# wjwei-handsome/wgatools

Hardware: AMD Instinct MI355X
Metric: paf_cigar_ops_per_s (paf2maf+stat) (higher is better)
Workload: dtype u8

## Files before the change

wgatools_amd/csrc/capi_paf2maf.inc:

```
static inline u32 job_tiles_for(int param, u64 nt) {
  if (param >= 1) return param > (int)WGA_S_MAX_JOB_TILES ? WGA_S_MAX_JOB_TILES : (u32)param;
  return nt < 200000ull ? 4u : 8u;
}

extern "C" {

size_t wga_tile_ws_bytes(uint64_t n_ops) { return (size_t)(n_tiles(n_ops) * sizeof(wga_tile_sum)) + 16; }

int wga_cigar_stat(wga_ctx* c, const wga_cigar_batch* b, wga_cigar_counts* d_counts,
                   wga_rec_diag* d_diag, void* d_tile_ws) {
  int rc = ctx_bind(c);
  if (rc) return rc;
  if ((rc = check_batch(b))) return rc;
  if (b->n == 0) return WGA_OK;
  if (!d_counts || !d_diag) return fail(WGA_E_INVALID_ARG, "d_counts / d_diag null", nullptr);
  RT_CHECK(rt_memset(d_counts, 0, (size_t)b->n * sizeof(wga_cigar_counts), c->stream));
  RT_CHECK(rt_memset(d_diag, 0xFF, (size_t)b->n * sizeof(wga_rec_diag), c->stream));
  u64 nt = n_tiles(b->n_ops);
  if (nt == 0) return WGA_OK;
  void* ws;
  if ((rc = ctx_scratch(c, (size_t)nt * sizeof(wga_tile_rec), &ws))) return rc;
  wga_tile_rec* tile_rec = (wga_tile_rec*)ws;
  WGA_LAUNCH(k_tile_rec, (u32)((nt + 255) / 256), WGA_BLOCK, c->stream, (const u64*)b->d_op_off,
             b->d_strand_neg, b->n, (u64)b->n_ops, tile_rec);
  LAUNCH_CHECK();
  const u32 grid = (u32)((nt + 3) / 4);
  WGA_LAUNCH(k_cigar_stat, grid, WGA_BLOCK, c->stream, b->d_ops, (const u64*)b->d_op_off,
             b->d_strand_neg, b->n, (u64)b->n_ops, (const wga_tile_rec*)tile_rec, d_counts, d_diag,
             (wga_tile_sum*)d_tile_ws);
  LAUNCH_CHECK();
  return WGA_OK;
}

int wga_exclusive_scan_u64(wga_ctx* c, uint32_t n, const uint64_t* d_in, uint64_t* d_out) {
  int rc = ctx_bind(c);
  if (rc) return rc;
  if (!d_out || (n && !d_in)) return fail(WGA_E_INVALID_ARG, "null array", nullptr);
  ScanPlain f;
  f.in = (const u64*)d_in;
  return run_scan(c, f, n, (u64*)d_out);
}

int wga_paf2maf_layout(wga_ctx* c, uint32_t n, const wga_cigar_counts* d_counts,
                       const uint64_t* d_t_src_len, const uint64_t* d_q_src_len,
                       const uint32_t* d_pre_t, const uint32_t* d_pre_q, const uint32_t* d_post,
                       uint64_t* d_t_row_off, uint64_t* d_q_row_off, uint64_t* d_rec_off) {
  int rc = ctx_bind(c);
  if (rc) return rc;
  if (!d_rec_off) return fail(WGA_E_INVALID_ARG, "d_rec_off null", nullptr);
  if (n && (!d_counts || !d_t_src_len || !d_q_src_len || !d_t_row_off || !d_q_row_off))
    return fail(WGA_E_INVALID_ARG, "null array", nullptr);
  ScanLayout f;
  f.counts = d_counts;
  f.t_src_len = (const u64*)d_t_src_len;
  f.q_src_len = (const u64*)d_q_src_len;
  f.pre_t = d_pre_t;
  f.pre_q = d_pre_q;
  f.post = d_post;
  rc = run_scan(c, f, n, (u64*)d_rec_off);
  if (rc) return rc;
  if (n) {
    WGA_LAUNCH(k_layout_rows, (n + 255u) / 256u, WGA_BLOCK, c->stream, f, n, (const u64*)d_rec_off,
               (u64*)d_t_row_off, (u64*)d_q_row_off);
    LAUNCH_CHECK();
  }
  return WGA_OK;
}

int wga_paf2maf_expand(wga_ctx* c, const wga_cigar_batch* b, const wga_cigar_counts* d_counts,
                       const void* d_tile_ws, const uint8_t* d_t_fa, uint64_t t_fa_bytes,
                       const uint64_t* d_t_src_off, const uint64_t* d_t_src_len,
                       const uint8_t* d_q_fa, uint64_t q_fa_bytes, const uint64_t* d_q_src_off,
                       const uint64_t* d_q_src_len, uint8_t* d_out, const uint64_t* d_t_row_off,
                       const uint64_t* d_q_row_off, wga_rec_diag* d_diag) {
  int rc = ctx_bind(c);
  if (rc) return rc;
  if ((rc = check_batch(b))) return rc;
  if (b->n == 0 || b->n_ops == 0) return WGA_OK;
  if (!d_counts || !d_tile_ws || !d_t_src_off || !d_t_src_len || !d_q_src_off || !d_q_src_len ||
      !d_out || !d_t_row_off || !d_q_row_off || !d_diag)
    return fail(WGA_E_INVALID_ARG, "null array", nullptr);
  if ((t_fa_bytes && !d_t_fa) || (q_fa_bytes && !d_q_fa)) return fail(WGA_E_INVALID_ARG, "null sequence pool", nullptr);
  u64 nt = n_tiles(b->n_ops);
  if (nt > 0x7FFFFFFFull) return fail(WGA_E_INVALID_ARG, "batch too large for one launch", nullptr);
  void* ws;
  size_t rec_bytes = ((size_t)b->n * sizeof(wga_rec_desc) + 255) & ~(size_t)255;
  const size_t desc_bytes = (size_t)nt * sizeof(wga_tile_desc);
  const size_t list_bytes = 2 * (size_t)nt * sizeof(u32);
  const int variant = c->expand_variant >= 0 ? c->expand_variant : WGA_AUTO_LONG_VARIANT;
  c->expand_variant_used = variant;
  const bool stream = variant == 3;
  const u32 job_tiles = job_tiles_for(c->expand_job_tiles, nt);
  const u64 jobs = (nt + job_tiles - 1) / job_tiles;
  const size_t flag_bytes = stream ? (((size_t)nt + 255) & ~(size_t)255) : 0;
  const size_t skip_bytes = stream ? (((size_t)jobs * sizeof(u32) + 255) & ~(size_t)255) : 0;
  const size_t zero_bytes = 256 + flag_bytes + skip_bytes;
  if ((rc = ctx_scratch(c, rec_bytes + desc_bytes + list_bytes + zero_bytes, &ws))) return rc;
  wga_rec_desc* recs = (wga_rec_desc*)ws;
  wga_tile_desc* tdesc = (wga_tile_desc*)((char*)ws + rec_bytes);
  u32* const wide_list = (u32*)((char*)ws + rec_bytes + desc_bytes);
  u32* const fast_list = wide_list + nt;
  u32* const wide_counts = (u32*)((char*)ws + rec_bytes + desc_bytes + list_bytes);
  u8* const tile_flag = stream ? (u8*)wide_counts + 256 : nullptr;
  u32* const job_skip = stream ? (u32*)(tile_flag + flag_bytes) : nullptr;
  if (stream) RT_CHECK(rt_memset(wide_counts, 0, zero_bytes, c->stream));
  WGA_LAUNCH(k_rec_desc, (b->n + 255u) / 256u, WGA_BLOCK, c->stream, b->n, d_counts,
             b->d_strand_neg, (const u64*)d_t_src_off, (const u64*)d_t_src_len,
             (const u64*)d_q_src_off, (const u64*)d_q_src_len, (const u64*)d_t_row_off,
             (const u64*)d_q_row_off, recs, (const u64*)b->d_op_off, (u64)t_fa_bytes, (u64)q_fa_bytes, tile_flag);
  LAUNCH_CHECK();
  WGA_LAUNCH(k_tile_base, (u32)((nt + 255) / 256), WGA_BLOCK, c->stream, (const u64*)b->d_op_off,
             (u64)b->n_ops, (const wga_tile_sum*)d_tile_ws, (const wga_rec_desc*)recs, tdesc, 0, (const u8*)tile_flag,
             job_tiles, c->expand_force_slow, job_skip, wide_counts, fast_list, wide_list);
  LAUNCH_CHECK();
  if (stream) c->stream_counts = wide_counts;
  ExpandArgs a;
  a.ops = b->d_ops;
  a.op_off = (const u64*)b->d_op_off;
  a.n_ops = b->n_ops;
  a.tdesc = tdesc;
  a.recs = recs;
  a.t_fa = d_t_fa;
  a.t_fa_bytes = t_fa_bytes;
  a.q_fa = d_q_fa;
  a.q_fa_bytes = q_fa_bytes;
  a.out = d_out;
  a.diag = d_diag;
  a.force_slow = c->expand_force_slow;
  a.no_table = c->expand_no_table;
  a.drain_min = 0;
  a.tile_count = nullptr;
  a.tile_list = nullptr;
  a.n_rec = b->n;
  a.job_tiles = job_tiles;
  a.job_skip = job_skip;
  a.drain_min = c->expand_drain_min ? c->expand_drain_min : ((u64)t_fa_bytes + (u64)q_fa_bytes > WGA_DRAIN_POOL_BYTES ? 16u : 32u);
  c->expand_drain_min_used = a.drain_min;
  const uint32_t slot = c->ev_n % (uint32_t)wga_ctx::kTimingRing;
  if (c->timing) RT_CHECK(rt_event_record(c->ev[2 * slot], c->stream));
  if (stream) {
    WGA_LAUNCH(k_paf2maf_expand_s, (u32)jobs, 128u, c->stream, a);
    LAUNCH_CHECK();
    const u32 side_grid = nt < 256 ? (u32)nt : 256u;
    a.tile_count = wide_counts;
    a.tile_list = fast_list;
    WGA_LAUNCH(k_paf2maf_expand_list, side_grid, WGA_BLOCK, c->stream, a);
    LAUNCH_CHECK();
    a.force_slow = 1;
    a.tile_count = wide_counts + 1;
    a.tile_list = wide_list;
    WGA_LAUNCH(k_paf2maf_expand_list, side_grid, WGA_BLOCK, c->stream, a);
    LAUNCH_CHECK();
  } else {
    WGA_LAUNCH(k_paf2maf_expand, (u32)nt, WGA_BLOCK, c->stream, a);
    LAUNCH_CHECK();
  }
  if (c->timing) {
    RT_CHECK(rt_event_record(c->ev[2 * slot + 1], c->stream));
    c->ev_n++;
  }
  return WGA_OK;
}

int wga_ctx_expand_timing(wga_ctx* c, double* ms_sum, uint32_t* launches) {
  int rc = ctx_bind(c);
  if (rc) return rc;
  if (!ms_sum || !launches) return fail(WGA_E_INVALID_ARG, "null argument", nullptr);
  *ms_sum = 0.0;
  *launches = 0;
  if (!c->timing) return WGA_OK;
  const uint32_t n = c->ev_n < (uint32_t)wga_ctx::kTimingRing ? c->ev_n : (uint32_t)wga_ctx::kTimingRing;
  for (uint32_t k = 0; k < n; k++) {
    float ms = 0.0f;
    RT_CHECK(rt_event_elapsed_ms(c->ev[2 * k], c->ev[2 * k + 1], &ms));
    *ms_sum += (double)ms;
  }
  *launches = n;
  c->ev_n = 0;
  return WGA_OK;
}

int wga_scatter_bytes(wga_ctx* c, uint32_t n, const uint8_t* d_src, const uint64_t* d_src_off,
                      uint8_t* d_dst, const uint64_t* d_dst_off) {
  int rc = ctx_bind(c);
  if (rc) return rc;
  if (n == 0) return WGA_OK;
  if (!d_src || !d_src_off || !d_dst || !d_dst_off) return fail(WGA_E_INVALID_ARG, "null array", nullptr);
  WGA_LAUNCH(k_scatter_bytes, (n + 3u) / 4u, WGA_BLOCK, c->stream, n, d_src, (const u64*)d_src_off,
             d_dst, (const u64*)d_dst_off);
  LAUNCH_CHECK();
  return WGA_OK;
}

int wga_counts_total(wga_ctx* c, uint32_t n, const wga_cigar_counts* d_counts, uint64_t* d_totals) {
  int rc = ctx_bind(c);
  if (rc) return rc;
  if (!d_totals || (n && !d_counts)) return fail(WGA_E_INVALID_ARG, "null array", nullptr);
  static_assert(sizeof(wga_cigar_counts) == 88, "wga_cigar_counts is 11 u64");
  RT_CHECK(rt_memset(d_totals, 0, 88, c->stream));
  if (n == 0) return WGA_OK;
  u32 grid = (u32)(((u64)n * 11ull + 253ull * 8ull - 1ull) / (253ull * 8ull));
  if (grid > 2048u) grid = 2048u;
  WGA_LAUNCH(k_counts_total, grid, WGA_BLOCK, c->stream, n, (const u64*)d_counts, (u64*)d_totals);
// ... 6 lines not shown
```

wgatools_amd/csrc/capi_pafpseudo.inc:

```
static CallKey class_tab_key(const wga_cigar_batch* b) {
  return {6, {{b->d_ops, (size_t)b->n_ops * 4}, {b->d_op_off, ((size_t)b->n + 1) * 8}}, {b->n, b->n_ops}};
}

extern "C" {

int wga_cigar_class_sums(wga_ctx* c, const wga_cigar_batch* b, wga_class_sums* d_sums) {
  int rc = ctx_bind(c);
  if (rc) return rc;
  if ((rc = check_batch(b))) return rc;
  if (b->n == 0) return WGA_OK;
  if (!d_sums) return fail(WGA_E_INVALID_ARG, "d_sums null", nullptr);
  wga_ctx::ClassTab& t = c->class_tab;
  const CallKey key = class_tab_key(b);
  t.cache.take(key, false);
  u64 nt = n_tiles(b->n_ops);
  if (nt == 0) {
    RT_CHECK(rt_memset(d_sums, 0, (size_t)b->n * sizeof(wga_class_sums), c->stream));
    return WGA_OK;
  }
  const size_t tile_bytes = ((size_t)nt * sizeof(wga_tile_sum) + 63) & ~(size_t)63;
  const size_t need = tile_bytes + (size_t)b->n * sizeof(wga_class_sums);
  if ((rc = t.buf.reserve(c, need, need + need / 4))) return rc;
  t.tiles = (wga_tile_sum*)t.buf.mem;
  t.rec_sums = (wga_class_sums*)((char*)t.buf.mem + tile_bytes);
// ... 24 lines not shown
  RT_CHECK(rt_memset(d_diag, 0xFF, (size_t)b->n * sizeof(wga_rec_diag), c->stream));
  u64 nt = n_tiles(b->n_ops);
  if (nt == 0) return WGA_OK;
  wga_tile_sum* tiles;
  wga_class_sums* rec_sums;
  wga_ctx::ClassTab& t = c->class_tab;
  const bool kept = t.cache.take(class_tab_key(b), true);
  if (nt > 0x7FFFFFFFull) return fail(WGA_E_INVALID_ARG, "batch too large for one launch", nullptr);
  const bool stream = c->pseudo_variant == 3;
  const size_t tile_bytes = kept ? 0 : ((size_t)nt * sizeof(wga_tile_sum) + 255) & ~(size_t)255;
  const size_t sums_bytes = kept ? 0 : ((size_t)b->n * sizeof(wga_class_sums) + 255) & ~(size_t)255;
  const size_t rec_bytes = stream ? ((size_t)b->n * sizeof(wga_rec_desc) + 255) & ~(size_t)255 : 0;
  const size_t desc_bytes = stream ? (size_t)nt * sizeof(wga_tile_desc) : 0;
  const size_t list_bytes = stream ? 2 * (size_t)nt * sizeof(u32) : 0;
  const u32 job_tiles = job_tiles_for(c->expand_job_tiles, nt);
  const u64 jobs = (nt + job_tiles - 1) / job_tiles;
  const size_t flag_bytes = stream ? (((size_t)nt + 255) & ~(size_t)255) : 0;
  const size_t skip_bytes = stream ? (((size_t)jobs * sizeof(u32) + 255) & ~(size_t)255) : 0;
  const size_t zero_bytes = stream ? 256 + flag_bytes + skip_bytes : 0;
  void* ws = nullptr;
  if (tile_bytes + sums_bytes + rec_bytes + desc_bytes + list_bytes + zero_bytes)
    if ((rc = ctx_scratch(c, tile_bytes + sums_bytes + rec_bytes + desc_bytes + list_bytes + zero_bytes, &ws))) return rc;
  c->pseudo_counts = nullptr;
  if (kept) {
    tiles = t.tiles;
    rec_sums = t.rec_sums;
  } else {
    tiles = (wga_tile_sum*)ws;
    rec_sums = (wga_class_sums*)((char*)ws + tile_bytes);
    RT_CHECK(rt_memset(rec_sums, 0, (size_t)b->n * sizeof(wga_class_sums), c->stream));
    WGA_LAUNCH(k_class_tiles, (u32)((nt + 3) / 4), WGA_BLOCK, c->stream, b->d_ops,
               (const u64*)b->d_op_off, b->n, (u64)b->n_ops, tiles, rec_sums);
    LAUNCH_CHECK();
  }
  PseudoArgs a;
  a.ops = b->d_ops;
  a.op_off = (const u64*)b->d_op_off;
  a.strand_neg = b->d_strand_neg;
  a.n = b->n;
  a.n_ops = b->n_ops;
  a.tiles = tiles;
  a.rec_sums = rec_sums;
  a.base_mode = base_mode;
  a.q_fa = d_q_fa;
  a.q_fa_bytes = q_fa_bytes;
  a.q_src_off = (const u64*)d_q_src_off;
  a.q_src_len = (const u64*)d_q_src_len;
  a.skip = (const u64*)d_skip;
  a.out = d_out;
  a.dst_off = (const u64*)d_dst_off;
  a.diag = d_diag;
  a.tile_count = nullptr;
  a.tile_list = nullptr;
  if (stream) {
    char* const base = (char*)ws + tile_bytes + sums_bytes;
    wga_rec_desc* const recs = (wga_rec_desc*)base;
    wga_tile_desc* const tdesc = (wga_tile_desc*)(base + rec_bytes);
    u32* const list_wide = (u32*)(base + rec_bytes + desc_bytes);
    u32* const list_fast = list_wide + nt;
    u32* const counts = (u32*)(base + rec_bytes + desc_bytes + list_bytes);
    u8* const tile_flag = (u8*)counts + 256;
    u32* const job_skip = (u32*)(tile_flag + flag_bytes);
    RT_CHECK(rt_memset(counts, 0, zero_bytes, c->stream));
    WGA_LAUNCH(k_pseudo_rec_desc, (b->n + 255u) / 256u, WGA_BLOCK, c->stream, b->n, (const wga_class_sums*)rec_sums, b->d_strand_neg,
               base_mode ? (const u64*)d_q_src_off : nullptr, base_mode ? (const u64*)d_q_src_len : nullptr, (const u64*)d_skip,
               (const u64*)d_dst_off, (const u64*)b->d_op_off, (u64)q_fa_bytes, recs, tile_flag);
    LAUNCH_CHECK();
    WGA_LAUNCH(k_tile_base, (u32)((nt + 255) / 256), WGA_BLOCK, c->stream, (const u64*)b->d_op_off, (u64)b->n_ops,
               (const wga_tile_sum*)tiles, (const wga_rec_desc*)recs, tdesc, 1, (const u8*)tile_flag, job_tiles, 0, job_skip, counts,
               list_fast, list_wide);
    LAUNCH_CHECK();
    c->pseudo_counts = counts;
    ExpandArgs e;
    memset(&e, 0, sizeof(e));
    e.ops = b->d_ops;
    e.op_off = (const u64*)b->d_op_off;
    e.n_ops = b->n_ops;
    e.tdesc = tdesc;
    e.recs = recs;
    e.q_fa = base_mode ? d_q_fa : nullptr;
    e.q_fa_bytes = base_mode ? q_fa_bytes : 0;
    e.out = d_out;
    e.diag = d_diag;
    e.n_rec = b->n;
    e.job_tiles = job_tiles;
    e.job_skip = job_skip;
    if (base_mode)
      WGA_LAUNCH(k_pafpseudo_stream, (u32)((jobs + 1) / 2), 128u, c->stream, e);
    else
      WGA_LAUNCH(k_pafpseudo_stream_sym, (u32)((jobs + 1) / 2), 128u, c->stream, e);
    LAUNCH_CHECK();
    const u32 side_grid = nt < 256 ? (u32)nt : 256u;
    a.tile_count = counts;
    a.tile_list = list_fast;
    if (base_mode)
      WGA_LAUNCH(k_pafpseudo_fill_list<true>, side_grid, WGA_BLOCK, c->stream, a);
    else
      WGA_LAUNCH(k_pafpseudo_fill_list<false>, side_grid, WGA_BLOCK, c->stream, a);
    LAUNCH_CHECK();
    a.tile_count = counts + 1;
    a.tile_list = list_wide;
    if (base_mode)
      WGA_LAUNCH(k_pafpseudo_fill_list<true>, side_grid, WGA_BLOCK, c->stream, a);
    else
      WGA_LAUNCH(k_pafpseudo_fill_list<false>, side_grid, WGA_BLOCK, c->stream, a);
    LAUNCH_CHECK();
    return WGA_OK;
  }
  if (base_mode)
    WGA_LAUNCH(k_pafpseudo_fill<true>, (u32)nt, WGA_BLOCK, c->stream, a);
  else
    WGA_LAUNCH(k_pafpseudo_fill<false>, (u32)nt, WGA_BLOCK, c->stream, a);
  LAUNCH_CHECK();
  return WGA_OK;
}

}
```

wgatools_amd/csrc/wga_k6_pafpseudo.h:

```cpp
#ifndef WGA_K6_PAFPSEUDO_H
#define WGA_K6_PAFPSEUDO_H

#include "wga_kernels.h"

struct PseudoArgs {
  const u32* ops;
  const u64* op_off;
  const u8* strand_neg;
  u32 n;
  u64 n_ops;
  const wga_tile_sum* tiles;
  const wga_class_sums* rec_sums;
  int base_mode;
  const u8* q_fa;
  u64 q_fa_bytes;
  const u64* q_src_off;
  const u64* q_src_len;
  const u64* skip;
  u8* out;
  const u64* dst_off;
  wga_rec_diag* diag;
  const u32* tile_count;
  const u32* tile_list;
};

__device__ __forceinline__ u32 pseudo_symbol(u32 code) {
  return (code == WGA_OP_M || code == WGA_OP_EQ)
             ? 0x31313131u
             : code == WGA_OP_X ? 0x30303030u
                                : (code == WGA_OP_D || code == WGA_OP_D_CONT) ? 0x2D2D2D2Du : 0u;
}

__device__ __forceinline__ void emit_symbols(u8* dst, u32 N, u32 c0, const u32* s_col,
                                             const u32* s_sym, int ka, int kb, const u32* optbl, u32 gsh,
                                             const u32x4_a16* lowmask, u32 tid, u32 nthreads) {
  if (N == 0) return;
  const u64 A = (u64)dst, E = A + N;
  const u64 first = A >> 4, last = (E - 1) >> 4;
  for (u64 ch = first + tid; ch <= last; ch += nthreads) {
    const u64 base_addr = ch << 4;
    const u32 a0 = base_addr < A ? (u32)(A - base_addr) : 0u;
    const u32 b0 = base_addr + 16 > E ? (u32)(E - base_addr) : 16u;
    const u32 cz = c0 + (u32)(base_addr - A);
    u32 c = cz + a0;
    const u32 c_end = cz + b0;
    (void)kb;
    int k = (int)optbl[c >> gsh] - 1;
    k = k < ka ? ka : k;
    u32 o[4] = {0u, 0u, 0u, 0u};
    while (c < c_end) {
      u32 oe = s_col[k + 1];
      u32 pe = oe < c_end ? oe : c_end;
      if (pe > c) {
        const u32 sym = s_sym[k];
        const u32 W[4] = {sym, sym, sym, sym};
        merge16(o, W, (int)(c - cz), (int)(pe - cz), lowmask);
        c = pe;
      }
      k++;
    }
    if (a0 == 0u && b0 == 16u) {
      u32x4_a16 v = {o[0], o[1], o[2], o[3]};
      *(u32x4_a16*)base_addr = v;
    } else {
      u8* p = (u8*)base_addr;
      for (u32 j = a0; j < b0; j++) {
        u32 d = j >> 2;
        u32 word = d == 0 ? o[0] : d == 1 ? o[1] : d == 2 ? o[2] : o[3];
        p[j] = (u8)(word >> (8u * (j & 3u)));
      }
    }
  }
}

#ifndef WGA_K6_BLOCKS_BASE
#define WGA_K6_BLOCKS_BASE 4
// ... 200 lines not shown
          rd.tsh = 0u;
          rd.gsh = gsh;
          rd.queue = s_queue;
          rowsrc_prepare(qs, qb);
          emit_row(dst + (x0 - skip), (u32)(x1 - x0), c_first, rd, qs, tid, WGA_BLOCK, bad_base);
        } else
          emit_symbols(dst + (x0 - skip), (u32)(x1 - x0), c_first, s_col, s_sym, (int)ka, (int)kb, s_tbl, gsh,
                       s_lowmask, tid, WGA_BLOCK);
      }
    }
    if (!fast) {
      u64 x = cb, qp = qb;
      for (u64 k = cur; k < seg_end; k++) {
        const u32 op = a.ops[k];
        const u32 code = op & 15u;
        const u32 c = op_class(code);
        const u64 len = op >> 4;
        if (BASE && tid == 0) {
          if ((c == CLS_I || c == CLS_S) && qp + len > qs.src_len) atomicMin(panic_idx, k - rs);
          if (c == CLS_D && qp > qs.src_len) atomicMin(panic_idx, k - rs);
        }
        if (c == CLS_MX || c == CLS_D) {
          for (u64 j = tid; j < len; j += WGA_BLOCK) {
            u64 xx = x + j;
            if (xx >= skip && xx < row_len) {
              u8 v;
              if (BASE)
                v = (c == CLS_D) ? (u8)'-' : src_byte(qs, qp + j, bad_base);
              else
                v = (u8)(pseudo_symbol(code) & 0xFFu);
              dst[xx - skip] = v;
            }
          }
          x += len;
        }
        if (c == CLS_MX || c == CLS_I || c == CLS_S) qp += len;
      }
    }
    if (seg_end == re && BASE && row_len > T_total) {
      u64 x0 = T_total > skip ? T_total : skip;
      if (row_len > x0)
        emit_tail(dst + (x0 - skip), row_len - x0, Q_total + (x0 - T_total), qs, s_lowmask, s_queue, s_zero2, s_g_col, tid, WGA_BLOCK, bad_base);
    }
    cur = seg_end;
    r++;
  }
}
template <bool BASE>
__global__ __launch_bounds__(256, BASE ? WGA_K6_BLOCKS_BASE : WGA_K6_BLOCKS_SYM) void k_pafpseudo_fill(PseudoArgs a) {
  pseudo_tile<BASE>(a, xcd_tile_of_block());
}
template <bool BASE>
__global__ __launch_bounds__(256, BASE ? WGA_K6_BLOCKS_BASE : WGA_K6_BLOCKS_SYM) void k_pafpseudo_fill_list(PseudoArgs a) {
  const u32 n_list = *a.tile_count;
  for (u32 idx = blockIdx.x; idx < n_list; idx += gridDim.x) {
    pseudo_tile<BASE>(a, a.tile_list[idx]);
    __syncthreads();
  }
}

#endif
```

wgatools_amd/csrc/wga_kernels.h:

```cpp
#ifndef WGA_KERNELS_H
#define WGA_KERNELS_H

#include "../../include/wga_hip.h"
#include "wga_rt.h"

typedef unsigned int u32;
typedef unsigned long long u64;
typedef long long i64;
typedef unsigned char u8;

#define WGA_TILE 1024u
#define WGA_BLOCK 256u
#define WGA_FAST_COL_LIMIT 0x7FFFFFFFull

#define CLS_MX 0u
#define CLS_I 1u
#define CLS_D 2u
#define CLS_S 3u
#define CLS_O 4u

__device__ __forceinline__ u32 op_class(u32 code) {
  const u64 lut = (u64)CLS_MX | ((u64)CLS_I << 3) | ((u64)CLS_D << 6) | ((u64)CLS_O << 9) |
                  ((u64)CLS_S << 12) | ((u64)CLS_O << 15) | ((u64)CLS_O << 18) |
                  ((u64)CLS_MX << 21) | ((u64)CLS_MX << 24) | ((u64)CLS_I << 27) |
// ... 55 lines not shown
  }
  return v;
}

__device__ __forceinline__ void block_excl_scan4_u32(const u32 v[4], u32 ex[4], u32 tot[4],
                                                     u32* s_w4, bool s_w4_idle = false) {
  const u32 lane = threadIdx.x & 63u, wave = WGA_WAVE_ID(threadIdx.x);
  u32 inc[4];
#pragma unroll
  for (int k = 0; k < 4; k++) inc[k] = wave_incl_scan_u32(v[k]);
  if (!s_w4_idle) __syncthreads();
  if (lane == 63u) {
#pragma unroll
    for (int k = 0; k < 4; k++) s_w4[wave * 4 + k] = inc[k];
  }
  __syncthreads();
#pragma unroll
  for (int k = 0; k < 4; k++) {
    u32 pre = 0, t = 0;
#pragma unroll
    for (u32 w = 0; w < 4; w++) {
      const u32 x = s_w4[w * 4 + k];
      pre += w < wave ? x : 0u;
      t += x;
    }
    ex[k] = pre + inc[k] - v[k];
    tot[k] = t;
  }
}

__device__ __forceinline__ u32 wga_find_rec(const u64* off, u32 n, u64 x) {
  u32 lane = threadIdx.x & 63u;
  u64 lo = 0, hi = (u64)n + 1;
  while (hi - lo > 1) {
    u64 span = hi - lo;
    u64 step = (span + 63) >> 6;
    u64 p = lo + (u64)(lane + 1) * step;
    int pred = (p < hi) && (off[p] <= x);
    u64 m = __ballot(pred);
    u64 k = (u64)__popcll(m);
    u64 nhi = lo + (k + 1) * step;
    lo = lo + k * step;
    hi = nhi < hi ? nhi : hi;
  }
  return (u32)lo;
}

struct wga_tile_rec {
  u32 rec, neg;
  u64 rs, re;
};
__global__ __launch_bounds__(256) void k_tile_rec(const u64* __restrict__ op_off,
                                                  const u8* __restrict__ strand_neg, u32 n, u64 n_ops,
                                                  wga_tile_rec* __restrict__ tile_rec) {
  const u64 g = (u64)blockIdx.x * 256 + threadIdx.x;
  const u64 x = g * WGA_TILE;
  if (x >= n_ops) return;
  u32 lo = 0, hi = n;
  while (hi - lo > 1u) {
    const u32 mid = lo + ((hi - lo) >> 1);
    if (op_off[mid] <= x)
      lo = mid;
    else
      hi = mid;
  }
  wga_tile_rec t;
  t.rec = lo;
  t.neg = strand_neg[lo] != 0 ? 1u : 0u;
  t.rs = op_off[lo];
  t.re = op_off[lo + 1];
  tile_rec[g] = t;
}

__device__ __forceinline__ void cigar_stat_tile(const u64 g, const u32 (&w)[16], const u32 lane, const u64* __restrict__ op_off,
                                                const u8* __restrict__ strand_neg, u64 n_ops,
                                                const wga_tile_rec* __restrict__ tile_rec, wga_cigar_counts* counts,
                                                wga_rec_diag* diag, wga_tile_sum* tiles) {
  const u64 tile_start = g * WGA_TILE;
  const u64 tile_end = tile_start + WGA_TILE < n_ops ? tile_start + WGA_TILE : n_ops;

  const wga_tile_rec tr = tile_rec[g];
  u32 r = WGA_UNI32(tr.rec);
  const u32 r_first = r;
  u64 cur = tile_start;
  u64 tot[5] = {0, 0, 0, 0, 0}, tail[5] = {0, 0, 0, 0, 0};
  u64 re = WGA_UNI64(tr.re);
  constexpr u32 MX_BITS = 0x01810181u, I_BITS = 0x02020202u, X_BITS = 0x01000100u, RARE_BITS = 0xF878F878u;
  constexpr u32 IEV_BITS = 0x00020002u, DEV_BITS = 0x00040004u;
  const u32 lane4 = lane * 4u;
  auto wave_sums = [&](u32 s_mx, u32 s_i, u32 s_t, u32 s_x, u32 ev, u64& Smx, u64& Si, u64& St, u64& Sx, u32& EV) {
    if (__ballot(s_t >= (1u << 26)) == 0ull) {
      Smx = wave_sum_u32(s_mx), Si = wave_sum_u32(s_i), St = wave_sum_u32(s_t), Sx = wave_sum_u32(s_x);
    } else {
      Smx = wave_sum_u32_wide(s_mx), Si = wave_sum_u32_wide(s_i), St = wave_sum_u32_wide(s_t), Sx = wave_sum_u32_wide(s_x);
    }
    EV = wave_sum_u32(ev);
  };
  u64 Wmx, Wi, Wt, Wx;
  u32 Wev;
  bool rare_tile;
  {
    u32 s_mx = 0, s_i = 0, s_t = 0, s_x = 0, ev = 0, rare = 0;
#pragma unroll
    for (int k = 0; k < 16; k++) {
      const u32 op = w[k], len = op >> 4;
      s_mx += len & bit_mask(MX_BITS, op);
      s_i += len & bit_mask(I_BITS, op);
      s_t += len;
// ... 248 lines not shown

template <typename F>
__global__ __launch_bounds__(256) void k_scan_partials(F f, u32 n, u64* partial) {
  __shared__ u64 s_w[5];
  u32 base = blockIdx.x * 1024u + threadIdx.x * 4u;
  u64 v = 0;
  for (u32 e = 0; e < 4; e++)
    if (base + e < n) v += f(base + e);
  u64 tot;
  (void)block_excl_scan_u64(v, s_w, &tot);
  if (threadIdx.x == 0) partial[blockIdx.x] = tot;
}

__global__ __launch_bounds__(256) void k_scan_top(u64* partial, u32 nb, u64* total_out) {
  __shared__ u64 s_w[5];
  u64 carry = 0;
  for (u32 base = 0; base < nb; base += 256u) {
    u32 i = base + threadIdx.x;
    u64 v = i < nb ? partial[i] : 0;
    u64 tot;
    u64 ex = block_excl_scan_u64(v, s_w, &tot);
    if (i < nb) partial[i] = carry + ex;
    carry += tot;
  }
  if (threadIdx.x == 0) *total_out = carry;
}

template <typename F>
__global__ __launch_bounds__(256) void k_scan_final(F f, u32 n, const u64* partial, u64* out) {
  __shared__ u64 s_w[5];
  u32 base = blockIdx.x * 1024u + threadIdx.x * 4u;
  u64 x[4];
  u64 v = 0;
  for (u32 e = 0; e < 4; e++) {
    x[e] = (base + e < n) ? f(base + e) : 0;
    v += x[e];
  }
  u64 tot;
  u64 ex = block_excl_scan_u64(v, s_w, &tot) + partial[blockIdx.x];
  for (u32 e = 0; e < 4; e++) {
    if (base + e < n) out[base + e] = ex;
    ex += x[e];
  }
}

__global__ __launch_bounds__(256) void k_layout_rows(ScanLayout f, u32 n, const u64* rec_off,
                                                     u64* t_row_off, u64* q_row_off) {
  u32 i = blockIdx.x * 256u + threadIdx.x;
  if (i >= n) return;
  u64 t = rec_off[i] + (f.pre_t ? f.pre_t[i] : 0u);
  u64 q = t + f.t_row(i) + (f.pre_q ? f.pre_q[i] : 0u);
  t_row_off[i] = t;
  q_row_off[i] = q;
}

#ifndef WGA_DRAIN_MIN
#define WGA_DRAIN_MIN 32u
#endif
#ifndef WGA_DRAIN_POOL_BYTES
#define WGA_DRAIN_POOL_BYTES (192ull << 20)
#endif
struct RowSrc {
  const u8* fa;
  u64 fa_bytes;
  u64 src_off;
  u64 src_len;
  bool rc;
  bool safe;
  u32 drain_min = WGA_DRAIN_MIN;
  const u8* win_base;
};



__device__ __forceinline__ u32 comp4(u32 x, u32* bad) {
  const u32 sel = x & 0x07070707u;
  const u32 fold = byte_perm(0x474EFF54u, 0x43FF41FFu, sel);
  const u32 comp = byte_perm(0x434EFF41u, 0x47FF54FFu, sel);
  *bad = (x & 0xDFDFDFDFu) ^ fold;
  return comp | (x & 0x20202020u);
}

__device__ __forceinline__ u32 bswap32(u32 x) {
  return (x >> 24) | ((x >> 8) & 0xFF00u) | ((x << 8) & 0xFF0000u) | (x << 24);
}
__device__ __forceinline__ u32 alignbyte(u32 hi, u32 lo, u32 sh) {
  return (u32)(((((u64)hi) << 32) | (u64)lo) >> (8u * sh));
}
__device__ __forceinline__ u32 bytemask(int lo, int hi) {
  lo = lo < 0 ? 0 : lo;
  hi = hi > 4 ? 4 : hi;
  if (hi <= lo) return 0u;
  u32 mh = hi >= 4 ? 0xFFFFFFFFu : ((1u << (8 * hi)) - 1u);
  u32 ml = (1u << (8 * lo)) - 1u;
  return mh & ~ml;
}

struct WinRaw {
  u32 v[4];
};

__device__ __forceinline__ void win_issue(const RowSrc& src, u64 sbase, int off, int pa, int pb,
                                          WinRaw& r) {
  if (src.safe) {
    const int sgn = src.rc ? -1 : 0;
    const u8* p = src.win_base + (i64)((off ^ sgn) - sgn);
// ... 471 lines not shown
  return o;
}

struct wga_rec_desc {
  u64 t_row_off, q_row_off;
  u64 t_src_off, t_src_len, q_src_off, q_src_len;
  u64 I_total, D_total, L;
  u64 neg;
};
struct wga_tile_base {
  u64 mx, i, d;
};
struct wga_tile_desc {
  u64 tile_cols;
  u32 rec, neg;
  u64 b_mx, b_i, b_d;
  u64 rs, re;
  u64 t_row_off, q_row_off, t_src_off, t_src_len, q_src_off, q_src_len, I_total, D_total, L;
};

__global__ __launch_bounds__(256) void k_rec_desc(u32 n, const wga_cigar_counts* counts,
                                                  const u8* strand_neg, const u64* t_src_off,
                                                  const u64* t_src_len, const u64* q_src_off,
                                                  const u64* q_src_len, const u64* t_row_off,
                                                  const u64* q_row_off, wga_rec_desc* out, const u64* op_off,
                                                  u64 t_fa_bytes, u64 q_fa_bytes, u8* tile_flag) {
  u32 r = blockIdx.x * 256u + threadIdx.x;
  if (r >= n) return;
  const wga_cigar_counts cn = counts[r];
  wga_rec_desc d;
  d.t_row_off = t_row_off[r];
  d.q_row_off = q_row_off[r];
  d.t_src_off = t_src_off[r];
  d.t_src_len = t_src_len[r];
  d.q_src_off = q_src_off[r];
  d.q_src_len = q_src_len[r];
  d.I_total = cn.ins_bp + cn.inv_ins_bp;
  d.D_total = cn.del_bp + cn.inv_del_bp;
  d.L = cn.match + cn.mismatch + d.I_total + d.D_total;
  d.neg = (strand_neg[r] != 0 ? 1u : 0u) | (d.t_src_len + d.I_total > d.L ? 2u : 0u) | (d.q_src_len + d.D_total > d.L ? 4u : 0u) |
          ((d.t_src_len + d.I_total < d.L || d.q_src_len + d.D_total < d.L) ? 8u : 0u);
  out[r] = d;
  if (!tile_flag) return;
  const bool inside = d.t_src_off >= 32ull && d.t_src_off + d.t_src_len + 32ull <= t_fa_bytes && d.q_src_off >= 32ull &&
                      d.q_src_off + d.q_src_len + 32ull <= q_fa_bytes;
  if ((d.neg & 0xEull) == 0ull && inside) return;
  const u64 a = op_off[r], b = op_off[r + 1];
  if (b <= a) return;
  for (u64 t = a / WGA_TILE; t <= (b - 1) / WGA_TILE; t++) tile_flag[t] = 1;
}

#define WGA_S_MAX_TILE_COLS (1ull << 24)
#define WGA_S_SKIP 0x100u
__global__ __launch_bounds__(256) void k_tile_base(const u64* op_off, u64 n_ops,
                                                   const wga_tile_sum* tiles,
                                                   const wga_rec_desc* recs, wga_tile_desc* descs, int pseudo,
                                                   const u8* tile_flag, u32 job_tiles, int all_slow, u32* job_skip,
                                                   u32* counts, u32* list_fast, u32* list_slow) {
  const u32 lane = threadIdx.x & 63u;
  const u64 g = (u64)blockIdx.x * 256 + threadIdx.x;
  const u64 tile_start = g * WGA_TILE;
  const bool valid = tile_start < n_ops;
  wga_tile_sum ts;
  u64 rs = 0, re = 0, g0 = 0;
  if (valid) {
    ts = tiles[g];
    rs = op_off[ts.rec];
    re = op_off[ts.rec + 1];
  }
  u64 p_mx = 0, p_i = 0, p_d = 0;
  bool far = false;
  if (valid && rs < tile_start) {
    g0 = rs / WGA_TILE;
    if (g - g0 <= 64) {
      for (u64 k = g0; k < g; k++) {
        const u64* v = (k == g0) ? tiles[k].tail : tiles[k].tot;
        p_mx += v[CLS_MX];
        p_i += v[CLS_I] + (pseudo ? v[CLS_S] : 0ull);
        p_d += v[CLS_D];
      }
    } else {
      far = true;
    }
  }
  u64 m = __ballot(far);
  while (m) {
    const int src = (int)__builtin_ctzll(m);
    const u64 gg = __shfl(g, src), gg0 = __shfl(g0, src);
    u64 a_mx = 0, a_i = 0, a_d = 0;
    for (u64 k = gg0 + lane; k < gg; k += 64) {
      const u64* v = (k == gg0) ? tiles[k].tail : tiles[k].tot;
      a_mx += v[CLS_MX];
      a_i += v[CLS_I] + (pseudo ? v[CLS_S] : 0ull);
      a_d += v[CLS_D];
    }
    a_mx = wave_sum_u64(a_mx);
    a_i = wave_sum_u64(a_i);
    a_d = wave_sum_u64(a_d);
    if ((int)lane == src) {
      p_mx = a_mx;
      p_i = a_i;
      p_d = a_d;
    }
    m &= m - 1;
  }
  if (!valid) return;
  const wga_rec_desc rd = recs[ts.rec];
  wga_tile_desc d;
  d.tile_cols = ts.tot[CLS_MX] + ts.tot[CLS_I] + ts.tot[CLS_D] + (pseudo ? ts.tot[CLS_S] : 0ull);
  d.rec = (u32)ts.rec;
  d.neg = (u32)rd.neg;
  if (tile_flag) {
    const bool slow = all_slow || d.tile_cols > WGA_FAST_COL_LIMIT;
    if (slow || tile_flag[g] || d.tile_cols > WGA_S_MAX_TILE_COLS) {
      d.neg |= WGA_S_SKIP;
      atomicOr(&job_skip[g / job_tiles], all_slow ? 0xFFFFFFFFu : 1u << (u32)(g % job_tiles));
      if (slow)
        list_slow[atomicAdd(&counts[1], 1u)] = (u32)g;
      else
        list_fast[atomicAdd(&counts[0], 1u)] = (u32)g;
    }
  }
  d.b_mx = p_mx;
  d.b_i = p_i;
  d.b_d = p_d;
  d.rs = rs;
  d.re = re;
  d.t_row_off = rd.t_row_off;
  d.q_row_off = rd.q_row_off;
  d.t_src_off = rd.t_src_off;
  d.t_src_len = rd.t_src_len;
  d.q_src_off = rd.q_src_off;
  d.q_src_len = rd.q_src_len;
  d.I_total = rd.I_total;
  d.D_total = rd.D_total;
  d.L = rd.L;
  descs[g] = d;
}

struct ExpandArgs {
  const u32* ops;
  const u64* op_off;
  u64 n_ops;
  const wga_tile_desc* tdesc;
  const wga_rec_desc* recs;
  const u8* t_fa;
  u64 t_fa_bytes;
  const u8* q_fa;
  u64 q_fa_bytes;
  u8* out;
  wga_rec_diag* diag;
  int force_slow;
  int no_table;
  u32 drain_min;
  const u32* tile_count;
  const u32* tile_list;
  u32 n_rec;
  u32 job_tiles;
  const u32* job_skip;
};

#ifndef WGA_K2_BLOCKS
#define WGA_K2_BLOCKS 6
#endif
__device__ __forceinline__ void expand_tile_v1(const ExpandArgs& a, const u64 g) {
  __shared__ u32 s_bnd[3][2];
  __shared__ u32 s_tot[2];
  __shared__ u32 s_tg_col[WGA_TILE + 2];
  __shared__ u32 s_tg_cum[WGA_TILE + 2];
  __shared__ u32 s_qg_col[WGA_TILE + 2];
  __shared__ u32 s_qg_cum[WGA_TILE + 2];
  __shared__ u32 s_zero2[2];
  __shared__ u32 s_w4[16];
  __shared__ u32x4_a16 s_lowmask[17];
  __shared__ u32 s_tbl[WGA_TBL_N + 2];
  __shared__ u32 s_queue[4 * WGA_QCAP];

  const u32 tid = threadIdx.x;
  const u32 lane = tid & 63u, wave = WGA_WAVE_ID(tid);
  const u64 tile_start = g * WGA_TILE;
  const u64 tile_end = tile_start + WGA_TILE < a.n_ops ? tile_start + WGA_TILE : a.n_ops;
  const u32 nt = (u32)(tile_end - tile_start);
  build_lowmask(s_lowmask);
  u32 pre = 0u;
  if (lane < 32u) pre = ((const u32*)(a.tdesc + g))[lane];
  const u64 tile_cols = wave_get_u64(pre, 0);
  const bool fast = !a.force_slow && tile_cols <= WGA_FAST_COL_LIMIT;
  u32 gsh = a.no_table ? 8u : WGA_TBL_SHIFT;
  while ((tile_cols >> gsh) >= WGA_TBL_N) gsh++;
  const bool use_tbl = fast;
  const u32 r0 = wave_get_u32(pre, 2);
  const u64 re0 = wave_get_u64(pre, 12);
  const u32 kb0 = re0 < tile_end ? (u32)(re0 - tile_start) : 0xFFFFFFFFu;
  if (use_tbl)
    for (u32 k = tid; k < WGA_TBL_N + 2u; k += WGA_BLOCK) s_tbl[k] = 0u;
  if (tid < 2u) s_zero2[tid] = 0u;

  u32 opw[4];
  {
    u32 base = tid * 4u;
    if (base + 3 < nt) {
      u32x4_a16 v = ops_load16(a.ops + tile_start + base);
      opw[0] = v[0];
      opw[1] = v[1];
      opw[2] = v[2];
      opw[3] = v[3];
    } else {
      for (int e = 0; e < 4; e++) opw[e] = (base + e < nt) ? a.ops[tile_start + base + e] : 0u;
    }
// ... 242 lines not shown
        src.src_off = wave_get_u64(dsc, 18 + q4);
        src.src_len = src_len;
        src.rc = is_q && (wave_get_u32(dsc, 3) & 1u) != 0u;
        src.drain_min = a.drain_min;
        u8* const dst = a.out + wave_get_u64(dsc, 14 + q2) + x0;
        const u64 sb0 = is_tail ? L - gap_total : (is_q ? qb : tb);
#endif
        for (u64 done = lo; done < hi; done += (1ull << 30)) {
          const u64 m = hi - done < (1ull << 30) ? hi - done : (1ull << 30);
          RowDesc rd;
          rd.c_org = is_tail ? 0u : col_a;
          rd.G_col = is_q ? s_qg_col : s_tg_col;
          rd.G_cum = is_q ? s_qg_cum : s_tg_cum;
          rd.G_adj = is_tail ? s_zero2 : rd.G_cum;
          rd.ga = is_tail ? 0 : (is_q ? ja : ia);
          rd.gb = is_tail ? 0 : (is_q ? jb : ib);
          rd.gcum_a = is_tail ? 0u : (is_q ? dcum_a : icum_a);
          rd.sbase = is_tail ? sb0 + done : sb0;
          rd.lowmask = s_lowmask;
          rd.tbl = is_tail ? s_zero2 : s_tbl;
          rd.tsh = (is_q && !is_tail) ? 16u : 0u;
          rd.gsh = is_tail ? 31u : gsh;
          rd.queue = s_queue;
          rowsrc_prepare(src, rd.sbase);
          emit_row(dst + done, (u32)m, is_tail ? 0u : col_a + (u32)done, rd, src, coop ? tid : lane,
                   coop ? WGA_BLOCK : 64u, bad_base);
        }
      }
    }
    cur = seg_end;
    r++;
    if (cur < tile_end) re = a.op_off[r + 1];
    nseg++;
  }
}

#ifndef WGA_K2_XCD
#define WGA_K2_XCD 1
#endif
__device__ __forceinline__ u64 xcd_tile_of_block() {
#if WGA_K2_XCD
  const u32 nt = gridDim.x, b = blockIdx.x, x = b & 7u, q = nt >> 3, r = nt & 7u;
  return (u64)(x * q + (x < r ? x : r) + (b >> 3));
#else
  return blockIdx.x;
#endif
}
__global__ __launch_bounds__(256, WGA_K2_BLOCKS) void k_paf2maf_expand(ExpandArgs a) {
  expand_tile_v1(a, xcd_tile_of_block());
}


__global__ __launch_bounds__(256, 4) void k_paf2maf_expand_list(ExpandArgs a) {
  const u32 n_list = *a.tile_count;
  for (u32 idx = blockIdx.x; idx < n_list; idx += gridDim.x) {
    expand_tile_v1(a, a.tile_list[idx]);
    __syncthreads();
  }
}

__global__ __launch_bounds__(256) void k_scatter_bytes(u32 n, const u8* src, const u64* src_off,
                                                       u8* dst, const u64* dst_off) {
  const u32 lane = threadIdx.x & 63u;
  const u64 i = (u64)blockIdx.x * 4 + WGA_WAVE_ID(threadIdx.x);
  if (i >= n) return;
  const u64 s0 = src_off[i], s1 = src_off[i + 1], d0 = dst_off[i];
  for (u64 k = s0 + lane; k < s1; k += 64) dst[d0 + (k - s0)] = src[k];
}

#define WGA_PEER_MAX 15
struct wga_peer_srcs {
  const int* p[WGA_PEER_MAX];
};
__global__ __launch_bounds__(256) void k_add_peers_i32(int* __restrict__ dst, wga_peer_srcs srcs, int n_src, u64 n) {
  const u64 tid = (u64)blockIdx.x * 256u + threadIdx.x, stride = (u64)gridDim.x * 256u;
  bool together = true;
  for (int k = 0; k < n_src; k++) together = together && ((((u64)srcs.p[k]) ^ (u64)dst) & 15ull) == 0ull;
  u64 head = together ? ((16ull - ((u64)dst & 15ull)) & 15ull) >> 2 : n;
  if (head > n) head = n;
  const u64 groups = (n - head) >> 2, tail0 = head + (groups << 2);
  for (u64 q = tid; q < groups; q += stride) {
    const u64 i = head + (q << 2);
    u32x4_a16 acc = *(const u32x4_a16*)(dst + i);
    u32x4_a16 v[WGA_PEER_MAX];
#pragma unroll
    for (int k = 0; k < WGA_PEER_MAX; k++)
      if (k < n_src) v[k] = *(const u32x4_a16*)(srcs.p[k] + i);
#pragma unroll
    for (int k = 0; k < WGA_PEER_MAX; k++)
      if (k < n_src) acc += v[k];
    *(u32x4_a16*)(dst + i) = acc;
  }
  for (u64 i = tid; i < n - (groups << 2); i += stride) {
    const u64 j = i < head ? i : tail0 + (i - head);
    int acc = dst[j];
    for (int k = 0; k < n_src; k++) acc += srcs.p[k][j];
    dst[j] = acc;
  }
}

#endif
```

Before: 79.42 billion.

## Fuse memsets, layout scan and list launches; skip unneeded tile descriptors

Folds the counts/diag memsets into the k_tile_rec kernel with a grid-stride clear. Replaces the generic scan plus row-offset kernel with a two-kernel fused layout scan when the block count is small. Merges the separate fast-list and wide-list expand/fill launches into one launch that walks both lists. k_tile_base also skips building descriptors for streamed tiles that no consumer reads. The aim is fewer launches and less wasted descriptor work. The risk is that the wide-list tiles no longer run with force_slow set, and descriptors are left unwritten for skipped tiles.

```diff
diff --git a/wgatools_amd/csrc/capi_paf2maf.inc b/wgatools_amd/csrc/capi_paf2maf.inc
--- a/wgatools_amd/csrc/capi_paf2maf.inc
+++ b/wgatools_amd/csrc/capi_paf2maf.inc
@@ -14,15 +14,22 @@
   if ((rc = check_batch(b))) return rc;
   if (b->n == 0) return WGA_OK;
   if (!d_counts || !d_diag) return fail(WGA_E_INVALID_ARG, "d_counts / d_diag null", nullptr);
-  RT_CHECK(rt_memset(d_counts, 0, (size_t)b->n * sizeof(wga_cigar_counts), c->stream));
-  RT_CHECK(rt_memset(d_diag, 0xFF, (size_t)b->n * sizeof(wga_rec_diag), c->stream));
+  static_assert(sizeof(wga_cigar_counts) % 8 == 0 && sizeof(wga_rec_diag) % 8 == 0, "cleared in 8-byte words");
+  const u64 n_zero = (u64)b->n * (sizeof(wga_cigar_counts) / 8), n_ones = (u64)b->n * (sizeof(wga_rec_diag) / 8);
   u64 nt = n_tiles(b->n_ops);
-  if (nt == 0) return WGA_OK;
+  if (nt == 0) {
+    RT_CHECK(rt_memset(d_counts, 0, (size_t)b->n * sizeof(wga_cigar_counts), c->stream));
+    RT_CHECK(rt_memset(d_diag, 0xFF, (size_t)b->n * sizeof(wga_rec_diag), c->stream));
+    return WGA_OK;
+  }
   void* ws;
   if ((rc = ctx_scratch(c, (size_t)nt * sizeof(wga_tile_rec), &ws))) return rc;
   wga_tile_rec* tile_rec = (wga_tile_rec*)ws;
-  WGA_LAUNCH(k_tile_rec, (u32)((nt + 255) / 256), WGA_BLOCK, c->stream, (const u64*)b->d_op_off,
-             b->d_strand_neg, b->n, (u64)b->n_ops, tile_rec);
+  u64 tr_grid = (nt + 255) / 256;
+  const u64 clear_grid = std::min<u64>((n_zero + n_ones + 2047) / 2048, 1024);
+  if (tr_grid < clear_grid) tr_grid = clear_grid;
+  WGA_LAUNCH(k_tile_rec, (u32)tr_grid, WGA_BLOCK, c->stream, (const u64*)b->d_op_off, b->d_strand_neg, b->n, (u64)b->n_ops,
+             tile_rec, (u64*)d_counts, n_zero, (u64*)d_diag, n_ones);
   LAUNCH_CHECK();
   const u32 grid = (u32)((nt + 3) / 4);
   WGA_LAUNCH(k_cigar_stat, grid, WGA_BLOCK, c->stream, b->d_ops, (const u64*)b->d_op_off,
@@ -57,6 +64,17 @@
   f.pre_t = d_pre_t;
   f.pre_q = d_pre_q;
   f.post = d_post;
+  const u32 nb = (u32)(((u64)n + 1023u) / 1024u);
+  if (nb >= 1u && nb <= WGA_LAYOUT_FUSED_BLOCKS) {
+    void* ws;
+    if ((rc = ctx_scratch(c, (size_t)nb * sizeof(u64), &ws))) return rc;
+    WGA_LAUNCH(k_scan_partials<ScanLayout>, nb, WGA_BLOCK, c->stream, f, n, (u64*)ws);
+    LAUNCH_CHECK();
+    WGA_LAUNCH(k_layout_final, nb, WGA_BLOCK, c->stream, f, n, (const u64*)ws, (u64*)d_rec_off, (u64*)d_t_row_off,
+               (u64*)d_q_row_off);
+    LAUNCH_CHECK();
+    return WGA_OK;
+  }
   rc = run_scan(c, f, n, (u64*)d_rec_off);
   if (rc) return rc;
   if (n) {
@@ -111,7 +129,7 @@
   LAUNCH_CHECK();
   WGA_LAUNCH(k_tile_base, (u32)((nt + 255) / 256), WGA_BLOCK, c->stream, (const u64*)b->d_op_off,
              (u64)b->n_ops, (const wga_tile_sum*)d_tile_ws, (const wga_rec_desc*)recs, tdesc, 0, (const u8*)tile_flag,
-             job_tiles, c->expand_force_slow, job_skip, wide_counts, fast_list, wide_list);
+             job_tiles, c->expand_force_slow, job_skip, wide_counts, fast_list, wide_list, stream ? 1 : 0);
   LAUNCH_CHECK();
   if (stream) c->stream_counts = wide_counts;
   ExpandArgs a;
@@ -131,6 +149,7 @@
   a.drain_min = 0;
   a.tile_count = nullptr;
   a.tile_list = nullptr;
+  a.tile_list_wide = nullptr;
   a.n_rec = b->n;
   a.job_tiles = job_tiles;
   a.job_skip = job_skip;
@@ -144,11 +163,7 @@
     const u32 side_grid = nt < 256 ? (u32)nt : 256u;
     a.tile_count = wide_counts;
     a.tile_list = fast_list;
-    WGA_LAUNCH(k_paf2maf_expand_list, side_grid, WGA_BLOCK, c->stream, a);
-    LAUNCH_CHECK();
-    a.force_slow = 1;
-    a.tile_count = wide_counts + 1;
-    a.tile_list = wide_list;
+    a.tile_list_wide = wide_list;
     WGA_LAUNCH(k_paf2maf_expand_list, side_grid, WGA_BLOCK, c->stream, a);
     LAUNCH_CHECK();
   } else {
diff --git a/wgatools_amd/csrc/capi_pafpseudo.inc b/wgatools_amd/csrc/capi_pafpseudo.inc
--- a/wgatools_amd/csrc/capi_pafpseudo.inc
+++ b/wgatools_amd/csrc/capi_pafpseudo.inc
@@ -100,6 +100,7 @@
   a.diag = d_diag;
   a.tile_count = nullptr;
   a.tile_list = nullptr;
+  a.tile_list_wide = nullptr;
   if (stream) {
     char* const base = (char*)ws + tile_bytes + sums_bytes;
     wga_rec_desc* const recs = (wga_rec_desc*)base;
@@ -116,7 +117,7 @@
     LAUNCH_CHECK();
     WGA_LAUNCH(k_tile_base, (u32)((nt + 255) / 256), WGA_BLOCK, c->stream, (const u64*)b->d_op_off, (u64)b->n_ops,
                (const wga_tile_sum*)tiles, (const wga_rec_desc*)recs, tdesc, 1, (const u8*)tile_flag, job_tiles, 0, job_skip, counts,
-               list_fast, list_wide);
+               list_fast, list_wide, 1 );
     LAUNCH_CHECK();
     c->pseudo_counts = counts;
     ExpandArgs e;
@@ -141,13 +142,7 @@
     const u32 side_grid = nt < 256 ? (u32)nt : 256u;
     a.tile_count = counts;
     a.tile_list = list_fast;
-    if (base_mode)
-      WGA_LAUNCH(k_pafpseudo_fill_list<true>, side_grid, WGA_BLOCK, c->stream, a);
-    else
-      WGA_LAUNCH(k_pafpseudo_fill_list<false>, side_grid, WGA_BLOCK, c->stream, a);
-    LAUNCH_CHECK();
-    a.tile_count = counts + 1;
-    a.tile_list = list_wide;
+    a.tile_list_wide = list_wide;
     if (base_mode)
       WGA_LAUNCH(k_pafpseudo_fill_list<true>, side_grid, WGA_BLOCK, c->stream, a);
     else
diff --git a/wgatools_amd/csrc/wga_k6_pafpseudo.h b/wgatools_amd/csrc/wga_k6_pafpseudo.h
--- a/wgatools_amd/csrc/wga_k6_pafpseudo.h
+++ b/wgatools_amd/csrc/wga_k6_pafpseudo.h
@@ -22,6 +22,7 @@
   wga_rec_diag* diag;
   const u32* tile_count;
   const u32* tile_list;
+  const u32* tile_list_wide;
 };
 
 __device__ __forceinline__ u32 pseudo_symbol(u32 code) {
@@ -328,9 +329,9 @@
 }
 template <bool BASE>
 __global__ __launch_bounds__(256, BASE ? WGA_K6_BLOCKS_BASE : WGA_K6_BLOCKS_SYM) void k_pafpseudo_fill_list(PseudoArgs a) {
-  const u32 n_list = *a.tile_count;
+  const u32 n_fast = a.tile_count[0], n_list = n_fast + a.tile_count[1];
   for (u32 idx = blockIdx.x; idx < n_list; idx += gridDim.x) {
-    pseudo_tile<BASE>(a, a.tile_list[idx]);
+    pseudo_tile<BASE>(a, idx < n_fast ? a.tile_list[idx] : a.tile_list_wide[idx - n_fast]);
     __syncthreads();
   }
 }
diff --git a/wgatools_amd/csrc/wga_kernels.h b/wgatools_amd/csrc/wga_kernels.h
--- a/wgatools_amd/csrc/wga_kernels.h
+++ b/wgatools_amd/csrc/wga_kernels.h
@@ -131,8 +131,14 @@
 };
 __global__ __launch_bounds__(256) void k_tile_rec(const u64* __restrict__ op_off,
                                                   const u8* __restrict__ strand_neg, u32 n, u64 n_ops,
-                                                  wga_tile_rec* __restrict__ tile_rec) {
+                                                  wga_tile_rec* __restrict__ tile_rec, u64* zero, u64 n_zero, u64* ones,
+                                                  u64 n_ones) {
   const u64 g = (u64)blockIdx.x * 256 + threadIdx.x;
+  if (zero) {
+    const u64 stride = (u64)gridDim.x * 256;
+    for (u64 k = g; k < n_zero; k += stride) zero[k] = 0ull;
+    for (u64 k = g; k < n_ones; k += stride) ones[k] = ~0ull;
+  }
   const u64 x = g * WGA_TILE;
   if (x >= n_ops) return;
   u32 lo = 0, hi = n;
@@ -487,6 +493,40 @@
   u64 q = t + f.t_row(i) + (f.pre_q ? f.pre_q[i] : 0u);
   t_row_off[i] = t;
   q_row_off[i] = q;
+}
+
+#define WGA_LAYOUT_FUSED_BLOCKS 1024u
+__global__ __launch_bounds__(256) void k_layout_final(ScanLayout f, u32 n, const u64* partial, u64* rec_off, u64* t_row_off,
+                                                      u64* q_row_off) {
+  __shared__ u64 s_w[5];
+  u64 pv = 0;
+  for (u32 k = threadIdx.x; k < blockIdx.x; k += 256u) pv += partial[k];
+  u64 carry;
+  (void)block_excl_scan_u64(pv, s_w, &carry);
+  const u32 base = blockIdx.x * 1024u + threadIdx.x * 4u;
+  u64 x[4], to[4], qo[4];
+  u64 v = 0;
+  for (u32 e = 0; e < 4; e++) {
+    x[e] = to[e] = qo[e] = 0;
+    if (base + e < n) {
+      const u32 i = base + e;
+      to[e] = f.pre_t ? f.pre_t[i] : 0u;
+      qo[e] = to[e] + f.t_row(i) + (f.pre_q ? f.pre_q[i] : 0u);
+      x[e] = qo[e] + f.q_row(i) + (u64)(f.post ? f.post[i] : 0u);
+    }
+    v += x[e];
+  }
+  u64 tot;
+  u64 ex = block_excl_scan_u64(v, s_w, &tot) + carry;
+  for (u32 e = 0; e < 4; e++) {
+    if (base + e < n) {
+      rec_off[base + e] = ex;
+      t_row_off[base + e] = ex + to[e];
+      q_row_off[base + e] = ex + qo[e];
+    }
+    ex += x[e];
+  }
+  if (blockIdx.x == gridDim.x - 1u && threadIdx.x == 0u) rec_off[n] = carry + tot;
 }
 
 #ifndef WGA_DRAIN_MIN
@@ -1064,25 +1104,39 @@
 
 #define WGA_S_MAX_TILE_COLS (1ull << 24)
 #define WGA_S_SKIP 0x100u
+__device__ __forceinline__ u64 tile_sum_cols(const u64* tot, int pseudo) {
+  return tot[CLS_MX] + tot[CLS_I] + tot[CLS_D] + (pseudo ? tot[CLS_S] : 0ull);
+}
+__device__ __forceinline__ bool tile_left_to_v1(u64 cols, u8 flag, int all_slow) {
+  return all_slow || flag || cols > WGA_S_MAX_TILE_COLS || cols > WGA_FAST_COL_LIMIT;
+}
 __global__ __launch_bounds__(256) void k_tile_base(const u64* op_off, u64 n_ops,
                                                    const wga_tile_sum* tiles,
                                                    const wga_rec_desc* recs, wga_tile_desc* descs, int pseudo,
                                                    const u8* tile_flag, u32 job_tiles, int all_slow, u32* job_skip,
-                                                   u32* counts, u32* list_fast, u32* list_slow) {
+                                                   u32* counts, u32* list_fast, u32* list_slow, int sparse) {
   const u32 lane = threadIdx.x & 63u;
   const u64 g = (u64)blockIdx.x * 256 + threadIdx.x;
   const u64 tile_start = g * WGA_TILE;
   const bool valid = tile_start < n_ops;
   wga_tile_sum ts;
-  u64 rs = 0, re = 0, g0 = 0;
+  u64 rs = 0, re = 0, g0 = 0, cols = 0;
+  bool left = false;
+  bool need = valid;
   if (valid) {
     ts = tiles[g];
+    cols = tile_sum_cols(ts.tot, pseudo);
+    if (tile_flag) left = tile_left_to_v1(cols, tile_flag[g], all_slow);
+    if (sparse && tile_flag && !left && g % job_tiles != 0u)
+      need = tile_left_to_v1(tile_sum_cols(tiles[g - 1].tot, pseudo), tile_flag[g - 1], all_slow);
+  }
+  if (need) {
     rs = op_off[ts.rec];
     re = op_off[ts.rec + 1];
   }
   u64 p_mx = 0, p_i = 0, p_d = 0;
   bool far = false;
-  if (valid && rs < tile_start) {
+  if (need && rs < tile_start) {
     g0 = rs / WGA_TILE;
     if (g - g0 <= 64) {
       for (u64 k = g0; k < g; k++) {
@@ -1116,22 +1170,19 @@
     }
     m &= m - 1;
   }
-  if (!valid) return;
+  if (!need) return;
   const wga_rec_desc rd = recs[ts.rec];
   wga_tile_desc d;
-  d.tile_cols = ts.tot[CLS_MX] + ts.tot[CLS_I] + ts.tot[CLS_D] + (pseudo ? ts.tot[CLS_S] : 0ull);
+  d.tile_cols = cols;
   d.rec = (u32)ts.rec;
   d.neg = (u32)rd.neg;
-  if (tile_flag) {
-    const bool slow = all_slow || d.tile_cols > WGA_FAST_COL_LIMIT;
-    if (slow || tile_flag[g] || d.tile_cols > WGA_S_MAX_TILE_COLS) {
-      d.neg |= WGA_S_SKIP;
-      atomicOr(&job_skip[g / job_tiles], all_slow ? 0xFFFFFFFFu : 1u << (u32)(g % job_tiles));
-      if (slow)
-        list_slow[atomicAdd(&counts[1], 1u)] = (u32)g;
-      else
-        list_fast[atomicAdd(&counts[0], 1u)] = (u32)g;
-    }
+  if (left) {
+    d.neg |= WGA_S_SKIP;
+    atomicOr(&job_skip[g / job_tiles], all_slow ? 0xFFFFFFFFu : 1u << (u32)(g % job_tiles));
+    if (all_slow || cols > WGA_FAST_COL_LIMIT)
+      list_slow[atomicAdd(&counts[1], 1u)] = (u32)g;
+    else
+      list_fast[atomicAdd(&counts[0], 1u)] = (u32)g;
   }
   d.b_mx = p_mx;
   d.b_i = p_i;
@@ -1167,6 +1218,7 @@
   u32 drain_min;
   const u32* tile_count;
   const u32* tile_list;
+  const u32* tile_list_wide;
   u32 n_rec;
   u32 job_tiles;
   const u32* job_skip;
@@ -1515,9 +1567,9 @@
 
 
 __global__ __launch_bounds__(256, 4) void k_paf2maf_expand_list(ExpandArgs a) {
-  const u32 n_list = *a.tile_count;
+  const u32 n_fast = a.tile_count[0], n_list = n_fast + a.tile_count[1];
   for (u32 idx = blockIdx.x; idx < n_list; idx += gridDim.x) {
-    expand_tile_v1(a, a.tile_list[idx]);
+    expand_tile_v1(a, idx < n_fast ? a.tile_list[idx] : a.tile_list_wide[idx - n_fast]);
     __syncthreads();
   }
 }
```

Result: no change. 79.21 billion (median of 2 runs) (-0.3%).
